# falcon-computing/falcon-genome

Hardware: AMD Instinct MI355X
Metric: PairHMM GCUPS + banded-SW GCUPS per GPU; end-to-end htc regions/sec at 8 GPUs (higher is better)
Workload: dtype fp32 (fp64 rescue)

## Files before the change

### falcon-genome_amd/csrc/phmm_cols.h

```cpp
#pragma once

namespace fcs {

constexpr int kColsClasses = 8;
constexpr int kColsMinR = 33;
__host__ __device__ constexpr int cols_C(int c) { return c == 0 ? 19 : 18 - c; }
__host__ __device__ constexpr int cols_hmax(int c) { return 16 * cols_C(c) - 1; }
__host__ __device__ inline int cols_class(int H) {
  for (int c = kColsClasses - 1; c >= 0; --c)
    if (H <= cols_hmax(c)) return c;
  return -1;
}
constexpr int kColsRing = 32;
constexpr int kColsChunks = 6;
constexpr int kColsChunkBytes = kColsRing * 4 * 16;
constexpr int kColsCapOff = kColsChunks * kColsChunkBytes;
constexpr int kColsTabOff = kColsCapOff + 4 * 8 * 8;
constexpr int kColsLds = kColsTabOff + 3 * 128 * 4;

__device__ __forceinline__ uint32_t vconst(uint32_t k) {
  uint32_t r;
  asm volatile("v_mov_b32 %0, %1" : "=v"(r) : "i"(k));
  return r;
}

struct ColsItem {
  float e1, e3, my, yy, mm, gm, mx, xx;
  uint32_t tlo, thi;
  float z;
};

__device__ __forceinline__ ColsItem cols_item(const PhmmTables<float>& tab, const RawRow& raw, int role, bool first,
                                              float ih) {
  ColsItem c;
  if (role == 2 || role == 3) {
    const RowP<float> q = row_params<float, false>(tab, raw);
    const float x0 = first ? ih * tab.dmatch[raw.gq & 127] : 1.f;
    const bool last = role == 3;
    c.e1 = q.e1 * x0;
    c.e3 = q.e3 * x0;
    c.my = last ? 0.f : q.my;
    c.yy = q.yy;
    c.mm = last ? 1.f : q.mm;
    c.gm = last ? 1.f : q.gm;
    c.mx = last ? 0.f : q.mx;
    c.xx = last ? 0.f : q.xx;
    const int bc = base_code((unsigned char)raw.rb);
    c.tlo = bc < 4 ? 1u << (8 * bc) : bc == 4 ? vconst(0x01010101u) : 0u;
    c.thi = 0x00000001u;
    c.z = 0.f;
  } else if (role == 4) {
    c.e1 = 1.f;
    c.e3 = 0.f;
    c.my = c.yy = c.mm = c.gm = 1.f;
    c.mx = c.xx = 0.f;
    c.tlo = vconst(0x01010101u);
    c.thi = vconst(0x00000101u);
    c.z = 0.f;
  } else {
    c.e1 = c.e3 = c.my = c.mm = c.gm = c.mx = c.xx = 0.f;
    c.yy = 1.f;
    c.tlo = c.thi = 0u;
    c.z = 1.f;
  }
  return c;
}

__device__ __forceinline__ void cols_put(unsigned char* smem, int slot, int seg, int h, const ColsItem& c) {
  float* const p = reinterpret_cast<float*>(smem + (seg * kColsRing + slot) * 16) + h;
  constexpr int F = kColsChunkBytes / 4;
  p[0] = c.e1;
  p[2] = c.e3;
  p[F] = c.my;
  p[F + 2] = c.yy;
  p[2 * F] = c.mm;
  p[2 * F + 2] = c.gm;
  p[3 * F] = c.mx;
  p[3 * F + 2] = c.xx;
  uint32_t* const q = reinterpret_cast<uint32_t*>(p);
  q[4 * F] = c.tlo;
  q[4 * F + 2] = c.thi;
  q[5 * F] = __float_as_uint(c.z);
  q[5 * F + 2] = __float_as_uint(c.z);
}

template <int NW>
__device__ __forceinline__ void cols_convert(const uint32_t (&raw)[NW + 1], int al, int i0, int H, uint32_t (&code)[NW],
                                             bool& other) {
#pragma unroll
  for (int d = 0; d < NW; ++d) {
    const uint32_t x = __builtin_amdgcn_alignbyte(raw[d + 1], raw[d], (uint32_t)al);
    const int rel = H - (i0 + 4 * d);
    const int nv = min(max(rel, 0), 4);
    const uint32_t vmask = nv >= 4 ? 0xFFFFFFFFu : (1u << (8 * nv)) - 1u;
    const uint32_t sel = (x >> 1) & vconst(0x07070707u);
    uint32_t c = __builtin_amdgcn_perm(vconst(0x04050505u), vconst(0x02030100u), sel);
    const uint32_t back = __builtin_amdgcn_perm(vconst(0x0000004Eu), vconst(0x54474341u), c);
    other |= ((back ^ x) & vmask) != 0u;
    c = (c & vmask) | (vconst(0x06060606u) & ~vmask);
    if (rel >= 0 && rel < 4) c = (c & ~(0xFFu << (8 * rel))) | (0x05u << (8 * rel));
    code[d] = c;
  }
}

template <int NW>
__device__ __forceinline__ void cols_load(const uint8_t* __restrict__ hb, int64_t ho, int H, int i0, uint32_t (&raw)[NW + 1],
                                          int& al) {
  const int64_t s = ho + i0;
  al = (int)(s & 3);
  const int64_t base = s - al;
  const uint32_t* const src = reinterpret_cast<const uint32_t*>(hb + base);
#pragma unroll
  for (int d = 0; d <= NW; ++d) raw[d] = (base + 4 * d < ho + H && H > 0) ? src[d] : 0u;
}

template <int C>
__global__ __launch_bounds__(64, 2) void phmm4_kernel(
    const PhmmDevBatch b, const int32_t* __restrict__ order, const int64_t* __restrict__ bounds, const int cls,
    const int K, const int tail_pairs, const PhmmTables<float> gtab, double* __restrict__ out,
    int32_t* __restrict__ rescue_list, unsigned long long* __restrict__ rescue_count, const float thr,
    const int use_rescue, int32_t* __restrict__ fb_list, unsigned long long* __restrict__ fb_count) {
  constexpr int NW = (C + 3) / 4;
  extern __shared__ __align__(16) unsigned char smem_raw[];
  const int lane = threadIdx.x;
  const int seg = lane >> 4;
  const int sl = lane & 15;
  const int sbase = lane & 48;
  const int th = sl >> 3, tk = sl & 7;
  const int i0 = sl * C;
  const int64_t cbeg = bounds[cls];
  const long long count = bounds[cls + 1] - cbeg;
  order += cbeg;
  PhmmTables<float> tab = gtab;
  {
    float* const t = reinterpret_cast<float*>(smem_raw + kColsTabOff);
    for (int i = lane; i < 128; i += 64) {
      t[i] = gtab.ph2pr[i];
      t[128 + i] = gtab.dmatch[i];
      t[256 + i] = gtab.dmis[i];
    }
    tab.ph2pr = t;
    tab.dmatch = t + 128;
    tab.dmis = t + 256;
  }
  const long long tailn = count < (long long)tail_pairs ? count : (long long)tail_pairs;
  const long long headn = count - tailn;
  const long long per = 8LL * K;
  const long long nb_head = (headn + per - 1) / per;
  const long long nbatch = nb_head + (tailn + 7) / 8;

  for (long long w = blockIdx.x; w < nbatch; w += gridDim.x) {
    const bool head = w < nb_head;
    const int Kb = head ? K : 1;
    const long long bstart = head ? w * per : headn + (w - nb_head) * 8;
    const long long bend = head ? min(headn, bstart + per) : min(count, bstart + 8);
    const long long idx = bstart + 2 * seg + th + 8LL * tk;
    const int pm = (tk < Kb && idx < bend) ? order[idx] : -1;
    int Rm = 0, Hm = 0;
    int64_t rom = 0, hom = 0;
    float Im = 0.f;
    if (pm >= 0) {
      const int ri = b.pair_read[pm], hi = b.pair_hap[pm];
      Rm = b.read_len[ri];
      Hm = b.hap_len[hi];
      rom = b.read_off[ri];
      hom = b.hap_off[hi];
      Im = tab.init_const / (float)Hm;
    }
    const int len = pm >= 0 ? Rm + 2 : 0;
    int incl = len;
#pragma unroll
    for (int d = 1; d < 8; d <<= 1) {
      const int v = __shfl_up(incl, d, 8);
      if (tk >= d) incl += v;
    }
    const int Gm = incl - len;
    const int totA = __builtin_amdgcn_ds_bpermute(4 * (sbase + 7), incl);
    const int totB = __builtin_amdgcn_ds_bpermute(4 * (sbase + 15), incl);
    const int nsteps = ((wave_max(max(totA, totB)) + 15) + 7) & ~7;
    int sb = sbase * 4;
    auto bp = [&](int v, int h, int k) {
      return __builtin_amdgcn_ds_bpermute(sb + 4 * (8 * h + min(k, 7)), v);
    };
    auto tG = [&](int h, int k) { return bp(Gm, h, k); };
    auto tR = [&](int h, int k) { return bp(Rm, h, k); };
    auto tH = [&](int h, int k) { return bp(Hm, h, k); };
    auto tP = [&](int h, int k) { return bp(pm, h, k); };
    auto tI = [&](int h, int k) { return __int_as_float(bp(__float_as_int(Im), h, k)); };
    auto t64 = [&](int64_t v, int h, int k) {
      const int lo = bp((int)v, h, k), hi = bp((int)(v >> 32), h, k);
      return (int64_t)(((uint64_t)(uint32_t)hi << 32) | (uint32_t)lo);
    };
    auto valid = [&](int h, int k) {
      const int pv = tP(h, k);
      return k < Kb && pv >= 0;
    };

    uint32_t cur[2][NW], nxt[2][NW];
    int nk[2], swr[2];
    unsigned other[2] = {0u, 0u};
    auto fetch_codes = [&](int h, int k, uint32_t (&dst)[NW]) {
      const bool ok = valid(h, k);
      const int Hk = tH(h, k);
      const int H = ok ? Hk : 0;
      const int64_t ho = t64(hom, h, k);
      uint32_t raw[NW + 1];
      int al;
      cols_load<NW>(b.hb, ok ? ho : 0, H, i0, raw, al);
      bool oth = false;
      cols_convert<NW>(raw, al, i0, H, dst, oth);
      const unsigned long long bal = __ballot(oth && ok);
      if (((bal >> sbase) & 0xFFFFull) != 0ull) other[h] |= 1u << k;
    };
#pragma unroll
    for (int h = 0; h < 2; ++h) {
#pragma unroll
      for (int d = 0; d < NW; ++d) cur[h][d] = 0x06060606u;
      fetch_codes(h, 0, nxt[h]);
      nk[h] = 0;
      swr[h] = valid(h, 0) ? tG(h, 0) : 0x3FFFFFFF;
    }
    int kc[2] = {0, 0};
    int cap[2], capp[2];
    auto load_cap = [&](int h) {
      const bool ok = valid(h, kc[h]);
      const int v = tG(h, kc[h]) + tR(h, kc[h]);
      cap[h] = ok ? v : -0x3FFFFFFF;
      capp[h] = tP(h, kc[h]);
    };
    load_cap(0);
    load_cap(1);

    int kp = 0;
    RawRow praw{-1, 0, 0, 0, 0, 0, 0};
    int prole = 0;
    float pih = 0.f;
    bool kok = false, nok = false;
    int kG = 0, kR = 0, nG = 0;
    float kI = 0.f;
    int64_t kro = 0;
    auto load_cursor = [&] {
      kok = valid(th, kp);
      kG = tG(th, kp);
      kR = tR(th, kp);
      kI = tI(th, kp);
      kro = t64(rom, th, kp);
      nok = valid(th, kp + 1);
      nG = tG(th, kp + 1);
    };
    load_cursor();
    auto stage_a = [&](int base) {
      const int g = base + tk;
      const bool adv = nok && g >= nG;
      if (__ballot(adv) != 0ull) {
        if (adv) ++kp;
        load_cursor();
      }
      const bool ok = kok;
      const int G = kG, R = kR;
      pih = kI;
      const int64_t ro = kro;
      const int r = g - G;
      int role = 0;
      if (ok && r >= 0 && r < R) role = r == R - 1 ? 3 : 2;
      else if (ok && r == R) role = 4;
      prole = role | (r == 0 ? 16 : 0);
      praw = (role == 2 || role == 3) ? load_raw(b, R, ro, r) : RawRow{-1, 0, 0, 0, 0, 0, 0};
    };
    auto stage_b = [&](int base) {
      cols_put(smem_raw, (base + tk) & (kColsRing - 1), seg, th,
               cols_item(tab, praw, prole & 15, (prole & 16) != 0, pih));
    };
    {
      ColsItem z = cols_item(tab, RawRow{-1, 0, 0, 0, 0, 0, 0}, 0, false, 0.f);
      cols_put(smem_raw, 16 + tk, seg, th, z);
      cols_put(smem_raw, 24 + tk, seg, th, z);
      stage_a(0);
      stage_b(0);
      stage_a(8);
    }

    pf2 Xn[C], In[C];
#pragma unroll
    for (int j = 0; j < C; ++j) {
      Xn[j] = pf2{1.f, 1.f};
      In[j] = pf2{0.f, 0.f};
    }
    pf2 dn = pf2{1.f, 1.f}, xo = pf2{1.f, 1.f}, xin = pf2{1.f, 1.f};
    const uint32_t segoff = (uint32_t)seg * (kColsRing * 16u) + lds_addr(smem_raw);

    for (int t0 = 0; t0 < nsteps; t0 += 8) {
      asm volatile("" : "+v"(sb));
#pragma unroll
      for (int h = 0; h < 2; ++h) {
        const bool ev = swr[h] + 16 <= t0 && nk[h] + 1 < Kb;
        if (__ballot(ev) != 0ull) {
          uint32_t tmp[NW];
          fetch_codes(h, nk[h] + 1, tmp);
          const bool vn = valid(h, nk[h] + 1);
          const int gn = tG(h, nk[h] + 1);
          if (ev) {
#pragma unroll
            for (int d = 0; d < NW; ++d) nxt[h][d] = tmp[d];
            ++nk[h];
            swr[h] = vn ? gn : 0x3FFFFFFF;
          }
        }
        if (swr[h] + 16 <= t0 && nk[h] + 1 >= Kb) swr[h] = 0x3FFFFFFF;
      }
      stage_b(t0 + 8);
      stage_a(t0 + 16);
#pragma unroll
      for (int h = 0; h < 2; ++h) {
        const bool adv = cap[h] >= 0 && cap[h] + 15 < t0;
        if (__ballot(adv) != 0ull) {
          if (adv) ++kc[h];
          load_cap(h);
        }
      }
      bool capo[2];
#pragma unroll
      for (int h = 0; h < 2; ++h) capo[h] = (other[h] >> kc[h]) & 1u;
      const int g0 = t0 - sl;
      const bool any_cap = __ballot(sl == 15 && ((unsigned)(cap[0] - g0) < 8u || (unsigned)(cap[1] - g0) < 8u)) != 0ull;
      unsigned swmask = 0u;
#pragma unroll
      for (int q = 0; q < 4; ++q)
#pragma unroll
        for (int h = 0; h < 2; ++h) {
          const int lo = __builtin_amdgcn_readlane(swr[h], 16 * q) - t0;
          if (lo < 8 && lo + 15 >= 0) {
            const int a = max(lo, 0), bnd = min(lo + 15, 7);
            swmask |= ((2u << bnd) - 1u) & ~((1u << a) - 1u);
          }
        }
      const uint32_t xs = (uint32_t)(g0 & (kColsRing - 1)) * 16u;
      const uint32_t capa = lds_addr(smem_raw) + kColsCapOff + seg * 64;

      auto step = [&](auto S_) {
        constexpr int S = decltype(S_)::value;
        const int g = g0 + S;
        if (swmask & (1u << S)) {
#pragma unroll
          for (int h = 0; h < 2; ++h) {
            const bool take = g == swr[h];
#pragma unroll
            for (int d = 0; d < NW; ++d) {
              uint32_t r;
              asm("v_cndmask_b32_e64 %0, %1, %2, %3" : "=v"(r) : "v"(cur[h][d]), "v"(nxt[h][d]), "s"(__ballot(take)));
              cur[h][d] = r;
            }
          }
        }
        asm volatile("" ::: "memory");
        const uint32_t pa = ((xs + (uint32_t)(S * 16)) & (uint32_t)((kColsRing - 1) * 16)) + segoff;
        typedef float f4 __attribute__((ext_vector_type(4)));
        typedef uint32_t u4 __attribute__((ext_vector_type(4)));
        auto ld4 = [&](int chunk) {
          return *reinterpret_cast<const __attribute__((address_space(3))) f4*>((uintptr_t)(pa + chunk * kColsChunkBytes));
        };
        const f4 r0 = ld4(0), r1 = ld4(1), r2 = ld4(2), r3 = ld4(3);
        const u4 cr = *reinterpret_cast<const __attribute__((address_space(3))) u4*>((uintptr_t)(pa + 4 * kColsChunkBytes));
        const pf2 z1 = *reinterpret_cast<const __attribute__((address_space(3))) pf2*>((uintptr_t)(pa + 5 * kColsChunkBytes));
        const pf2 z2 = *reinterpret_cast<const __attribute__((address_space(3))) pf2*>((uintptr_t)(pa + 5 * kColsChunkBytes + 8));
        const pf2 e1 = pf2{r0.x, r0.y}, e3 = pf2{r0.z, r0.w}, my = pf2{r1.x, r1.y}, yy = pf2{r1.z, r1.w};
        const pf2 mm = pf2{r2.x, r2.y}, gm = pf2{r2.z, r2.w}, mx = pf2{r3.x, r3.y}, xx = pf2{r3.z, r3.w};
        pf2 din, xnx;
        din.x = __int_as_float(__builtin_amdgcn_update_dpp(__float_as_int(z1.x), __float_as_int(dn.x), kDppRowShr1, 0xF, 0xF, false));
        din.y = __int_as_float(__builtin_amdgcn_update_dpp(__float_as_int(z1.y), __float_as_int(dn.y), kDppRowShr1, 0xF, 0xF, false));
        xnx.x = __int_as_float(__builtin_amdgcn_update_dpp(__float_as_int(z2.x), __float_as_int(xo.x), kDppRowShr1, 0xF, 0xF, false));
        xnx.y = __int_as_float(__builtin_amdgcn_update_dpp(__float_as_int(z2.y), __float_as_int(xo.y), kDppRowShr1, 0xF, 0xF, false));
        const pf2 xcur = xin;
        xin = xnx;
        uint32_t mA = 0, mB = 0;
        auto prior = [&](int j, const pf2 dep) {
          if ((j & 3) == 0) {
            mA = __builtin_amdgcn_perm(cr.z, cr.x, cur[0][j >> 2]);
            mB = __builtin_amdgcn_perm(cr.w, cr.y, cur[1][j >> 2]);
          }
          int a, c;
          asm volatile("v_bfe_i32 %0, %2, %3, 1\n\tv_bfe_i32 %1, %4, %3, 1"
                       : "=&v"(a), "=&v"(c)
                       : "v"(mA), "i"(8 * (j & 3)), "v"(mB), "v"(dep));
          return pf2{sel_v((uint32_t)a, e1.x, e3.x), sel_v((uint32_t)c, e1.y, e3.y)};
        };
        pf2 Mn = xcur * prior(0, xcur);
        pf2 D = din, Mp = pf2{0.f, 0.f}, Dp = pf2{0.f, 0.f};
#pragma unroll
        for (int j = 0; j < C; ++j) {
          const pf2 M = Mn;
          if (j > 0) D = __builtin_elementwise_fma(Mp, my, Dp * yy);
          pf2 I = In[j], Xo = Xn[j];
          asm volatile("" : "+v"(I), "+v"(Xo) : "v"(D));
          if (j + 1 < C) Mn = Xo * prior(j + 1, D);
          pf2 xn = __builtin_elementwise_fma(M, mm, __builtin_elementwise_fma(I, gm, D));
          pf2 in = __builtin_elementwise_fma(M, mx, I * xx);
          asm volatile("" : "+v"(xn), "+v"(in));
          Xn[j] = xn;
          In[j] = in;
          Mp = M;
          Dp = D;
        }
        dn = __builtin_elementwise_fma(Mp, my, Dp * yy);
        xo = Xn[C - 1];
        uint64_t keep;
        const uint32_t cpa = capa + 0u;
        const pf2 dnv = dn;
        asm volatile(
            "s_mov_b64 %0, exec\n\t"
            "s_mov_b64 exec, %3\n\t"
            "ds_write_b64 %1, %2 offset:%4\n\t"
            "s_mov_b64 exec, %0"
            : "=&s"(keep)
            : "v"(cpa), "v"(dnv), "s"(kTopLanes), "i"(8 * S)
            : "memory");
      };
      [&]<int... S>(std::integer_sequence<int, S...>) {
        (step(std::integral_constant<int, S>{}), ...);
      }(std::make_integer_sequence<int, 8>{});
      if (any_cap) {
#pragma unroll
        for (int h = 0; h < 2; ++h)
          if (sl == 15 && (unsigned)(cap[h] - g0) < 8u) {
            const pf2 v = *reinterpret_cast<const pf2*>(smem_raw + kColsCapOff + seg * 64 + 8 * (cap[h] - g0));
            const float acc = h ? v.y : v.x;
            const int p = capp[h];
            if (capo[h]) {
              const unsigned long long k = atomicAdd(fb_count, 1ull);
              fb_list[k] = p;
              out[p] = __builtin_nan("");
            } else if (use_rescue && acc < thr) {
              const unsigned long long k = atomicAdd(rescue_count, 1ull);
              rescue_list[k] = p;
              out[p] = __builtin_nan("");
            } else {
              out[p] = (double)(log10f(acc) - tab.log10_init);
            }
          }
      }
    }
  }
}

constexpr int kCols1Ring = 48;
constexpr int kCols1Chunks = 5;
constexpr int kCols1ChunkBytes = kCols1Ring * 4 * 8;
constexpr int kCols1CapOff = kCols1Chunks * kCols1ChunkBytes;
constexpr int kCols1TabOff = kCols1CapOff + 4 * 16 * 4;
constexpr int kCols1Lds = kCols1TabOff + 3 * 128 * 4;
constexpr int kCols1MaxK = 16;
__host__ __device__ constexpr int cols1_waves(int C) { return 3; }
static_assert(kCols1Lds <= 10240, "16 waves per CU");

typedef uint32_t pu2 __attribute__((ext_vector_type(2)));

__device__ __forceinline__ void cols1_put(unsigned char* smem, int slot, int seg, const ColsItem& c) {
  unsigned char* const p = smem + (seg * kCols1Ring + slot) * 8;
  *reinterpret_cast<pf2*>(p) = pf2{c.e1, c.e3};
  *reinterpret_cast<pf2*>(p + kCols1ChunkBytes) = pf2{c.my, c.yy};
  *reinterpret_cast<pf2*>(p + 2 * kCols1ChunkBytes) = pf2{c.mm, c.gm};
  *reinterpret_cast<pf2*>(p + 3 * kCols1ChunkBytes) = pf2{c.mx, c.xx};
  *reinterpret_cast<pu2*>(p + 4 * kCols1ChunkBytes) = pu2{c.tlo, c.thi | (c.z != 0.f ? 0x01000000u : 0u)};
}

constexpr int kNever = 0x3FFFFFFF;

struct Cols1Seg {
  int pm, Rm, Hm, Gm;
  int64_t rom, hom;
  float Im;
};

__device__ __forceinline__ PhmmTables<float> cols1_tables(const PhmmTables<float>& gtab) {
  extern __shared__ __align__(16) unsigned char smem_raw[];
  PhmmTables<float> tab = gtab;
  float* const t = reinterpret_cast<float*>(smem_raw + kCols1TabOff);
  for (int i = threadIdx.x; i < 128; i += 64) {
    t[i] = gtab.ph2pr[i];
    t[128 + i] = gtab.dmatch[i];
    t[256 + i] = gtab.dmis[i];
  }
  tab.ph2pr = t;
  tab.dmatch = t + 128;
  tab.dmis = t + 256;
  return tab;
}

struct Cols1Batch {
  static constexpr bool kQueue = false;
  int Kb, nsteps;
  static __device__ __forceinline__ int slot(int k) { return min(k, 15); }
  static __device__ __forceinline__ int bit(int k) { return k; }
  __device__ __forceinline__ bool more(int t0) const { return t0 < nsteps; }
  __device__ __forceinline__ bool done(int) const { return false; }
};

constexpr int kCols6Lds = kCols1Lds;
constexpr int kCols6Waves = 3;
constexpr int kCols6Ahead = 48;
static_assert(kCols6Lds <= 13653, "12 waves per CU");

struct Cols1Queue {
  static constexpr bool kQueue = true;
  const int32_t* order;
  long long count;
  unsigned long long* qhead;
  unsigned pend;
  uint32_t qv;
  int nq = 0, gend = 0;
  bool closed = false;
  static __device__ __forceinline__ int slot(int k) { return k & 15; }
  static __device__ __forceinline__ int bit(int k) { return k & 15; }
  __device__ __forceinline__ bool more(int) const { return true; }
  __device__ __forceinline__ bool done(int kc) const { return __ballot(!closed || kc < nq) == 0ull; }
  __device__ __forceinline__ void complete(int gmin, const PhmmDevBatch& b, const PhmmTables<float>& tab, Cols1Seg& tb,
                                           unsigned& other) {
    const int seg = threadIdx.x >> 4, sl = threadIdx.x & 15;
    const long long base = (long long)(uint32_t)__builtin_amdgcn_readfirstlane((int)qv);
    const bool mine = (pend >> seg) & 1u;
    const long long idx = base + __popc(pend & ((1u << seg) - 1u));
    const bool got = mine && idx < count;
    if (mine && !got) closed = true;
    if (got) {
      const int p = order[idx];
      const int ri = b.pair_read[p], hi = b.pair_hap[p];
      const int R = b.read_len[ri], H = b.hap_len[hi];
      const int G = max(gend, gmin);
      if (sl == (nq & 15)) {
        tb.pm = p;
        tb.Rm = R;
        tb.Hm = H;
        tb.rom = b.read_off[ri];
        tb.hom = b.hap_off[hi];
        tb.Im = tab.init_const / (float)H;
        tb.Gm = G;
      }
      other &= ~(1u << (nq & 15));
      gend = G + R + 2;
      ++nq;
    }
    pend = 0u;
  }
  __device__ __forceinline__ void request(int t0, int kc) {
    const bool need = !closed && gend < t0 + 32 + kCols6Ahead && nq - kc < 8;
    const unsigned long long bal = __ballot(need && (threadIdx.x & 15) == 0);
    if (bal != 0ull) {
      pend = (unsigned)((bal & 1ull) | ((bal >> 15) & 2ull) | ((bal >> 30) & 4ull) | ((bal >> 45) & 8ull));
      qv = 0u;
      if (threadIdx.x == 0) qv = (uint32_t)atomicAdd(qhead, (unsigned long long)__popc(pend));
    }
  }
};

template <int C, class Feed>
__device__ __forceinline__ void cols1_stream(const PhmmDevBatch& b, const PhmmTables<float>& tab, Cols1Seg tb,
                                             Feed feed, double* __restrict__ out,
                                             int32_t* __restrict__ rescue_list,
                                             unsigned long long* __restrict__ rescue_count, const float thr,
                                             const int use_rescue, int32_t* __restrict__ fb_list,
                                             unsigned long long* __restrict__ fb_count) {
  constexpr int NW = (C + 3) / 4;
  extern __shared__ __align__(16) unsigned char smem_raw[];
  const int lane = threadIdx.x;
  const int seg = lane >> 4;
  const int sl = lane & 15;
  const int sbase = lane & 48;
  const int i0 = sl * C;
  int sb = sbase * 4;
  auto bp = [&](int v, int k) { return __builtin_amdgcn_ds_bpermute(sb + 4 * Feed::slot(k), v); };
  auto tG = [&](int k) { return bp(tb.Gm, k); };
  auto tR = [&](int k) { return bp(tb.Rm, k); };
  auto tH = [&](int k) { return bp(tb.Hm, k); };
  auto tP = [&](int k) { return bp(tb.pm, k); };
  auto tI = [&](int k) { return __int_as_float(bp(__float_as_int(tb.Im), k)); };
  auto t64 = [&](int64_t v, int k) {
    const int lo = bp((int)v, k), hi = bp((int)(v >> 32), k);
    return (int64_t)(((uint64_t)(uint32_t)hi << 32) | (uint32_t)lo);
  };
  auto valid = [&](int k) {
    if constexpr (Feed::kQueue) {
      return k >= 0 && k < feed.nq;
    } else {
      const int pv = tP(k);
      return k < feed.Kb && pv >= 0;
    }
  };

  uint32_t cur[NW], nxt[NW];
  int nk = -1, swr = kNever;
  unsigned other = 0u;
  auto fetch_codes = [&](int k, uint32_t (&dst)[NW]) {
    const bool ok = valid(k);
    const int Hk = tH(k);
    const int H = ok ? Hk : 0;
    const int64_t ho = t64(tb.hom, k);
    uint32_t raw[NW + 1];
    int al;
    cols_load<NW>(b.hb, ok ? ho : 0, H, i0, raw, al);
    bool oth = false;
    cols_convert<NW>(raw, al, i0, H, dst, oth);
    const unsigned long long bal = __ballot(oth && ok);
    if (((bal >> sbase) & 0xFFFFull) != 0ull) other |= 1u << Feed::bit(k);
  };
#pragma unroll
  for (int d = 0; d < NW; ++d) cur[d] = nxt[d] = 0x06060606u;
  int kc = 0, cap, capp;
  auto load_cap = [&] {
    const bool ok = valid(kc);
    const int v = tG(kc) + tR(kc);
    cap = ok ? v : -kNever;
    capp = tP(kc);
  };

  int kp = 0;
  RawRow praw{-1, 0, 0, 0, 0, 0, 0};
  int prole = 0;
  float pih = 0.f;
  bool kok = false, nok = false;
  int kG = 0, kR = 0, nG = 0;
  float kI = 0.f;
  int64_t kro = 0;
  auto load_cursor = [&] {
    kok = valid(kp);
    kG = tG(kp);
    kR = tR(kp);
    kI = tI(kp);
    kro = t64(tb.rom, kp);
    nok = valid(kp + 1);
    nG = tG(kp + 1);
  };
  auto stage_a = [&](int base) {
    const int g = base + sl;
    const bool adv = nok && g >= nG;
    if (__ballot(adv) != 0ull) {
      if (adv) ++kp;
      load_cursor();
    }
    const int r = g - kG;
    int role = 0;
    if (kok && r >= 0 && r < kR) role = r == kR - 1 ? 3 : 2;
    else if (kok && r == kR) role = 4;
    pih = kI;
    prole = role | (r == 0 ? 16 : 0);
    praw = (role == 2 || role == 3) ? load_raw(b, kR, kro, r) : RawRow{-1, 0, 0, 0, 0, 0, 0};
  };
  auto stage_b = [&](int base) {
    cols1_put(smem_raw, (int)((unsigned)(base + sl) % (unsigned)kCols1Ring), seg,
              cols_item(tab, praw, prole & 15, (prole & 16) != 0, pih));
  };
  if constexpr (Feed::kQueue) {
    feed.complete(0, b, tab, tb, other);
  } else {
    fetch_codes(0, nxt);
    nk = 0;
    swr = valid(0) ? tG(0) : kNever;
  }
  load_cursor();
  load_cap();
  {
    cols1_put(smem_raw, 32 + sl, seg, cols_item(tab, RawRow{-1, 0, 0, 0, 0, 0, 0}, 0, false, 0.f));
    stage_a(0);
    stage_b(0);
    stage_a(16);
  }

  float Xn[C], In[C];
#pragma unroll
  for (int j = 0; j < C; ++j) {
    Xn[j] = 1.f;
    In[j] = 0.f;
  }
  float dn = 1.f, xo = 1.f, xin = 1.f;
  const uint32_t segoff = (uint32_t)seg * (kCols1Ring * 8u) + lds_addr(smem_raw);

  for (int t0 = 0; feed.more(t0); t0 += 16) {
    asm volatile("" : "+v"(sb));
    if constexpr (Feed::kQueue) {
      if (feed.pend != 0u) {
        feed.complete(t0 + 32, b, tab, tb, other);
        load_cursor();
        load_cap();
      }
      feed.request(t0, kc);
    }
    {
      bool ev;
      if constexpr (Feed::kQueue) {
        if (swr != kNever && swr + 16 <= t0) swr = kNever;
        ev = swr == kNever && nk + 1 < feed.nq;
      } else {
        ev = swr + 16 <= t0 && nk + 1 < feed.Kb;
      }
      if (__ballot(ev) != 0ull) {
        uint32_t tmp[NW];
        fetch_codes(nk + 1, tmp);
        const bool vn = valid(nk + 1);
        const int gn = tG(nk + 1);
        if (ev) {
#pragma unroll
          for (int d = 0; d < NW; ++d) nxt[d] = tmp[d];
          ++nk;
          swr = vn ? gn : kNever;
        }
      }
      if constexpr (!Feed::kQueue)
        if (swr + 16 <= t0 && nk + 1 >= feed.Kb) swr = kNever;
    }
    stage_b(t0 + 16);
    stage_a(t0 + 32);
    {
      const bool adv = cap >= 0 && cap + 15 < t0;
      if (__ballot(adv) != 0ull) {
        if (adv) ++kc;
        load_cap();
      }
    }
    if (feed.done(kc)) break;
    const bool capo = (other >> Feed::bit(kc)) & 1u;
    const int gb = t0 - sl;
    const bool any_cap = __ballot(sl == 15 && (unsigned)(cap - gb) < 16u) != 0ull;
    unsigned swmask = 0u;
#pragma unroll
    for (int q = 0; q < 4; ++q) {
      const int lo = __builtin_amdgcn_readlane(swr, 16 * q) - t0;
      if (lo < 16 && lo + 15 >= 0) {
        const int a = max(lo, 0), bnd = min(lo + 15, 15);
        swmask |= ((2u << bnd) - 1u) & ~((1u << a) - 1u);
      }
    }
    uint32_t xs = ((uint32_t)(gb + kCols1Ring) % (uint32_t)kCols1Ring) * 8u;
    uint32_t capa = lds_addr(smem_raw) + kCols1CapOff + seg * 64;
    int g0 = gb;

#pragma nounroll
    for (int pass = 0; pass < 2; ++pass) {
      auto step = [&](auto S_) {
        constexpr int S = decltype(S_)::value;
        const int g = g0 + S;
        if (swmask & (1u << S)) {
          const bool take = g == swr;
#pragma unroll
          for (int d = 0; d < NW; ++d) {
            uint32_t r;
            asm("v_cndmask_b32_e64 %0, %1, %2, %3" : "=v"(r) : "v"(cur[d]), "v"(nxt[d]), "s"(__ballot(take)));
            cur[d] = r;
          }
        }
        asm volatile("" ::: "memory");
        const uint32_t a0 = xs + (uint32_t)(S * 8);
        const uint32_t pa = min(a0, a0 - (uint32_t)(kCols1Ring * 8)) + segoff;
        auto ld2 = [&](int chunk) {
          return *reinterpret_cast<const __attribute__((address_space(3))) pf2*>((uintptr_t)(pa + chunk * kCols1ChunkBytes));
        };
        const pf2 r0 = ld2(0), r1 = ld2(1), r2 = ld2(2), r3 = ld2(3);
        const pu2 cr = *reinterpret_cast<const __attribute__((address_space(3))) pu2*>((uintptr_t)(pa + 4 * kCols1ChunkBytes));
        const float e1 = r0.x, e3 = r0.y, my = r1.x, yy = r1.y, mm = r2.x, gm = r2.y, mx = r3.x, xx = r3.y;
        const float z = (float)(cr.y >> 24);
        const float din = __int_as_float(__builtin_amdgcn_update_dpp(__float_as_int(z), __float_as_int(dn), kDppRowShr1, 0xF, 0xF, false));
        const float xnx = __int_as_float(__builtin_amdgcn_update_dpp(__float_as_int(z), __float_as_int(xo), kDppRowShr1, 0xF, 0xF, false));
        const float xcur = xin;
        xin = xnx;
        uint32_t mA = 0;
        auto prior = [&](int j, const float dep) {
          if ((j & 3) == 0) mA = __builtin_amdgcn_perm(cr.y, cr.x, cur[j >> 2]);
          int a;
          asm volatile("v_bfe_i32 %0, %1, %2, 1" : "=v"(a) : "v"(mA), "i"(8 * (j & 3)), "v"(dep));
          return sel_v((uint32_t)a, e1, e3);
        };
        float Mn = xcur * prior(0, xcur);
        float D = din, Mp = 0.f, Dp = 0.f;
#pragma unroll
        for (int j = 0; j < C; ++j) {
          const float M = Mn;
          if (j > 0) D = __builtin_fmaf(Mp, my, Dp * yy);
          float I = In[j], Xo = Xn[j];
          asm volatile("" : "+v"(I), "+v"(Xo) : "v"(D));
          if (j + 1 < C) Mn = Xo * prior(j + 1, D);
          float xn = __builtin_fmaf(M, mm, __builtin_fmaf(I, gm, D));
          float in = __builtin_fmaf(M, mx, I * xx);
          asm volatile("" : "+v"(xn), "+v"(in));
          Xn[j] = xn;
          In[j] = in;
          Mp = M;
          Dp = D;
        }
        dn = __builtin_fmaf(Mp, my, Dp * yy);
        xo = Xn[C - 1];
        uint64_t keep;
        const uint32_t cpa = capa + 0u;
        const float dnv = dn;
        asm volatile(
            "s_mov_b64 %0, exec\n\t"
            "s_mov_b64 exec, %3\n\t"
            "ds_write_b32 %1, %2 offset:%4\n\t"
            "s_mov_b64 exec, %0"
            : "=&s"(keep)
            : "v"(cpa), "v"(dnv), "s"(kTopLanes), "i"(4 * S)
            : "memory");
      };
      [&]<int... S>(std::integer_sequence<int, S...>) {
        (step(std::integral_constant<int, S>{}), ...);
      }(std::make_integer_sequence<int, 8>{});
      g0 += 8;
      swmask >>= 8;
      capa += 32;
      xs += 64;
      xs = min(xs, xs - (uint32_t)(kCols1Ring * 8));
    }
    if (any_cap) {
      if (sl == 15 && (unsigned)(cap - gb) < 16u) {
        const float acc = *reinterpret_cast<const float*>(smem_raw + kCols1CapOff + seg * 64 + 4 * (cap - gb));
        const int p = capp;
        if (capo) {
          const unsigned long long k = atomicAdd(fb_count, 1ull);
          fb_list[k] = p;
          out[p] = __builtin_nan("");
        } else if (use_rescue && acc < thr) {
          const unsigned long long k = atomicAdd(rescue_count, 1ull);
          rescue_list[k] = p;
          out[p] = __builtin_nan("");
        } else {
          out[p] = (double)(log10f(acc) - tab.log10_init);
        }
      }
    }
  }
}

template <int C>
__global__ __launch_bounds__(64, cols1_waves(C)) void phmm5_kernel(
    const PhmmDevBatch b, const int32_t* __restrict__ order, const int64_t* __restrict__ bounds, const int cls,
    const int K, const int tail_pairs, const PhmmTables<float> gtab, double* __restrict__ out,
    int32_t* __restrict__ rescue_list, unsigned long long* __restrict__ rescue_count, const float thr,
    const int use_rescue, int32_t* __restrict__ fb_list, unsigned long long* __restrict__ fb_count) {
  const int lane = threadIdx.x;
  const int seg = lane >> 4;
  const int sl = lane & 15;
  const int sbase = lane & 48;
  const int64_t cbeg = bounds[cls];
  const long long count = bounds[cls + 1] - cbeg;
  order += cbeg;
  const PhmmTables<float> tab = cols1_tables(gtab);
  const long long tailn = count < (long long)tail_pairs ? count : (long long)tail_pairs;
  const long long headn = count - tailn;
  const long long per = 4LL * K;
  const long long nb_head = (headn + per - 1) / per;
  const long long nbatch = nb_head + (tailn + 3) / 4;

  for (long long w = blockIdx.x; w < nbatch; w += gridDim.x) {
    const bool head = w < nb_head;
    const int Kb = head ? K : 1;
    const long long bstart = head ? w * per : headn + (w - nb_head) * 4;
    const long long bend = head ? min(headn, bstart + per) : min(count, bstart + 4);
    const long long idx = bstart + seg + 4LL * sl;
    Cols1Seg tb{(sl < Kb && idx < bend) ? order[idx] : -1, 0, 0, 0, 0, 0, 0.f};
    if (tb.pm >= 0) {
      const int ri = b.pair_read[tb.pm], hi = b.pair_hap[tb.pm];
      tb.Rm = b.read_len[ri];
      tb.Hm = b.hap_len[hi];
      tb.rom = b.read_off[ri];
      tb.hom = b.hap_off[hi];
      tb.Im = tab.init_const / (float)tb.Hm;
    }
    const int len = tb.pm >= 0 ? tb.Rm + 2 : 0;
    int incl = len;
#pragma unroll
    for (int d = 1; d < 16; d <<= 1) {
      const int v = __shfl_up(incl, d, 16);
      if (sl >= d) incl += v;
    }
    tb.Gm = incl - len;
    const int tot = __builtin_amdgcn_ds_bpermute(4 * (sbase + 15), incl);
    const int nsteps = ((wave_max(tot) + 15) + 15) & ~15;
    cols1_stream<C>(b, tab, tb, Cols1Batch{Kb, nsteps}, out, rescue_list, rescue_count, thr, use_rescue, fb_list,
                    fb_count);
  }
}

template <int C>
__global__ __launch_bounds__(64, kCols6Waves) void phmm6_kernel(
    const PhmmDevBatch b, const int32_t* __restrict__ order, const int64_t* __restrict__ bounds, const int cls,
    const PhmmTables<float> gtab, double* __restrict__ out, int32_t* __restrict__ rescue_list,
    unsigned long long* __restrict__ rescue_count, const float thr, const int use_rescue,
    int32_t* __restrict__ fb_list, unsigned long long* __restrict__ fb_count,
    unsigned long long* __restrict__ qhead) {
  const int64_t cbeg = bounds[cls];
  const long long count = bounds[cls + 1] - cbeg;
  uint32_t qv = 0u;
  if (threadIdx.x == 0) qv = (uint32_t)atomicAdd(qhead, 4ull);
  if ((long long)(uint32_t)__builtin_amdgcn_readfirstlane((int)qv) >= count) return;
  const PhmmTables<float> tab = cols1_tables(gtab);
  cols1_stream<C>(b, tab, Cols1Seg{-1, 0, 0, 0, 0, 0, 0.f}, Cols1Queue{order + cbeg, count, qhead, 0xFu, qv}, out,
                  rescue_list, rescue_count, thr, use_rescue, fb_list, fb_count);
}

}
```

Measured before the change: 4584.

## Rescale PairHMM column recurrence by mm to drop one multiply per cell

```diff
diff --git a/falcon-genome_amd/csrc/phmm_cols.h b/falcon-genome_amd/csrc/phmm_cols.h
--- a/falcon-genome_amd/csrc/phmm_cols.h
+++ b/falcon-genome_amd/csrc/phmm_cols.h
@@ -25,24 +25,30 @@
 }
 
 struct ColsItem {
-  float e1, e3, my, yy, mm, gm, mx, xx;
+  float e1, e3, b, yy, a, mx, xx;
   uint32_t tlo, thi;
   float z;
 };
 
-__device__ __forceinline__ ColsItem cols_item(const PhmmTables<float>& tab, const RawRow& raw, int role, bool first,
-                                              float ih) {
+constexpr float kColsMinMm = 0.0625f;
+
+__device__ __forceinline__ ColsItem cols_item(const PhmmTables<float>& tab, const RawRow& raw, int oiq, int role,
+                                              bool first, float ih, bool& hazard) {
   ColsItem c;
+  hazard = false;
   if (role == 2 || role == 3) {
     const RowP<float> q = row_params<float, false>(tab, raw);
-    const float x0 = first ? ih * tab.dmatch[raw.gq & 127] : 1.f;
+    const int oi = oiq & 127, od = raw.dq & 127;
+    const int hi = oi > od ? oi : od, lo = oi > od ? od : oi;
+    const float x0 = first ? ih * tab.dmatch[raw.gq & 127] : tab.mm[((hi * (hi + 1)) >> 1) + lo];
     const bool last = role == 3;
+    hazard = !last && !(q.mm >= kColsMinMm);
+    const float inv = (last || hazard) ? 0.f : 1.f / q.mm;
     c.e1 = q.e1 * x0;
     c.e3 = q.e3 * x0;
-    c.my = last ? 0.f : q.my;
+    c.b = q.my * inv;
     c.yy = q.yy;
-    c.mm = last ? 1.f : q.mm;
-    c.gm = last ? 1.f : q.gm;
+    c.a = last ? 1.f : q.gm * inv;
     c.mx = last ? 0.f : q.mx;
     c.xx = last ? 0.f : q.xx;
     const int bc = base_code((unsigned char)raw.rb);
@@ -52,14 +58,14 @@
   } else if (role == 4) {
     c.e1 = 1.f;
     c.e3 = 0.f;
-    c.my = c.yy = c.mm = c.gm = 1.f;
-    c.mx = c.xx = 0.f;
+    c.yy = 1.f;
+    c.a = c.b = c.mx = c.xx = 0.f;
     c.tlo = vconst(0x01010101u);
     c.thi = vconst(0x00000101u);
     c.z = 0.f;
   } else {
-    c.e1 = c.e3 = c.my = c.mm = c.gm = c.mx = c.xx = 0.f;
-    c.yy = 1.f;
+    c.e1 = c.e3 = c.a = c.mx = c.xx = 0.f;
+    c.b = c.yy = 1.f;
     c.tlo = c.thi = 0u;
     c.z = 1.f;
   }
@@ -71,10 +77,10 @@
   constexpr int F = kColsChunkBytes / 4;
   p[0] = c.e1;
   p[2] = c.e3;
-  p[F] = c.my;
+  p[F] = c.b;
   p[F + 2] = c.yy;
-  p[2 * F] = c.mm;
-  p[2 * F + 2] = c.gm;
+  p[2 * F] = c.a;
+  p[2 * F + 2] = 0.f;
   p[3 * F] = c.mx;
   p[3 * F + 2] = c.xx;
   uint32_t* const q = reinterpret_cast<uint32_t*>(p);
@@ -266,13 +272,23 @@
       else if (ok && r == R) role = 4;
       prole = role | (r == 0 ? 16 : 0);
       praw = (role == 2 || role == 3) ? load_raw(b, R, ro, r) : RawRow{-1, 0, 0, 0, 0, 0, 0};
+      if (role == 2 || role == 3) prole |= (int)b.iq[ro + r] << 8;
     };
     auto stage_b = [&](int base) {
+      bool hz;
       cols_put(smem_raw, (base + tk) & (kColsRing - 1), seg, th,
-               cols_item(tab, praw, prole & 15, (prole & 16) != 0, pih));
+               cols_item(tab, praw, prole >> 8, prole & 15, (prole & 16) != 0, pih, hz));
+      if (__ballot(hz) != 0ull) {
+        unsigned m = hz ? 1u << (kp + 8 * th) : 0u;
+#pragma unroll
+        for (int d = 1; d < 16; d <<= 1) m |= (unsigned)__shfl_xor((int)m, d, 16);
+        other[0] |= m & 0xFFu;
+        other[1] |= m >> 8;
+      }
     };
     {
-      ColsItem z = cols_item(tab, RawRow{-1, 0, 0, 0, 0, 0, 0}, 0, false, 0.f);
+      bool hz;
+      ColsItem z = cols_item(tab, RawRow{-1, 0, 0, 0, 0, 0, 0}, 0, 0, false, 0.f, hz);
       cols_put(smem_raw, 16 + tk, seg, th, z);
       cols_put(smem_raw, 24 + tk, seg, th, z);
       stage_a(0);
@@ -363,8 +379,8 @@
         const u4 cr = *reinterpret_cast<const __attribute__((address_space(3))) u4*>((uintptr_t)(pa + 4 * kColsChunkBytes));
         const pf2 z1 = *reinterpret_cast<const __attribute__((address_space(3))) pf2*>((uintptr_t)(pa + 5 * kColsChunkBytes));
         const pf2 z2 = *reinterpret_cast<const __attribute__((address_space(3))) pf2*>((uintptr_t)(pa + 5 * kColsChunkBytes + 8));
-        const pf2 e1 = pf2{r0.x, r0.y}, e3 = pf2{r0.z, r0.w}, my = pf2{r1.x, r1.y}, yy = pf2{r1.z, r1.w};
-        const pf2 mm = pf2{r2.x, r2.y}, gm = pf2{r2.z, r2.w}, mx = pf2{r3.x, r3.y}, xx = pf2{r3.z, r3.w};
+        const pf2 e1 = pf2{r0.x, r0.y}, e3 = pf2{r0.z, r0.w}, cb = pf2{r1.x, r1.y}, yy = pf2{r1.z, r1.w};
+        const pf2 ca = pf2{r2.x, r2.y}, mx = pf2{r3.x, r3.y}, xx = pf2{r3.z, r3.w};
         pf2 din, xnx;
         din.x = __int_as_float(__builtin_amdgcn_update_dpp(__float_as_int(z1.x), __float_as_int(dn.x), kDppRowShr1, 0xF, 0xF, false));
         din.y = __int_as_float(__builtin_amdgcn_update_dpp(__float_as_int(z1.y), __float_as_int(dn.y), kDppRowShr1, 0xF, 0xF, false));
@@ -385,23 +401,23 @@
           return pf2{sel_v((uint32_t)a, e1.x, e3.x), sel_v((uint32_t)c, e1.y, e3.y)};
         };
         pf2 Mn = xcur * prior(0, xcur);
-        pf2 D = din, Mp = pf2{0.f, 0.f}, Dp = pf2{0.f, 0.f};
+        pf2 E = din, Mp = pf2{0.f, 0.f}, Ep = pf2{0.f, 0.f};
 #pragma unroll
         for (int j = 0; j < C; ++j) {
           const pf2 M = Mn;
-          if (j > 0) D = __builtin_elementwise_fma(Mp, my, Dp * yy);
+          if (j > 0) E = __builtin_elementwise_fma(Ep, yy, Mp);
           pf2 I = In[j], Xo = Xn[j];
-          asm volatile("" : "+v"(I), "+v"(Xo) : "v"(D));
-          if (j + 1 < C) Mn = Xo * prior(j + 1, D);
-          pf2 xn = __builtin_elementwise_fma(M, mm, __builtin_elementwise_fma(I, gm, D));
+          asm volatile("" : "+v"(I), "+v"(Xo) : "v"(E));
+          if (j + 1 < C) Mn = Xo * prior(j + 1, E);
+          pf2 xn = __builtin_elementwise_fma(E, cb, __builtin_elementwise_fma(I, ca, M));
           pf2 in = __builtin_elementwise_fma(M, mx, I * xx);
           asm volatile("" : "+v"(xn), "+v"(in));
           Xn[j] = xn;
           In[j] = in;
           Mp = M;
-          Dp = D;
+          Ep = E;
         }
-        dn = __builtin_elementwise_fma(Mp, my, Dp * yy);
+        dn = __builtin_elementwise_fma(Ep, yy, Mp);
         xo = Xn[C - 1];
         uint64_t keep;
         const uint32_t cpa = capa + 0u;
@@ -457,8 +473,8 @@
 __device__ __forceinline__ void cols1_put(unsigned char* smem, int slot, int seg, const ColsItem& c) {
   unsigned char* const p = smem + (seg * kCols1Ring + slot) * 8;
   *reinterpret_cast<pf2*>(p) = pf2{c.e1, c.e3};
-  *reinterpret_cast<pf2*>(p + kCols1ChunkBytes) = pf2{c.my, c.yy};
-  *reinterpret_cast<pf2*>(p + 2 * kCols1ChunkBytes) = pf2{c.mm, c.gm};
+  *reinterpret_cast<pf2*>(p + kCols1ChunkBytes) = pf2{c.b, c.yy};
+  *reinterpret_cast<pf2*>(p + 2 * kCols1ChunkBytes) = pf2{c.a, 0.f};
   *reinterpret_cast<pf2*>(p + 3 * kCols1ChunkBytes) = pf2{c.mx, c.xx};
   *reinterpret_cast<pu2*>(p + 4 * kCols1ChunkBytes) = pu2{c.tlo, c.thi | (c.z != 0.f ? 0x01000000u : 0u)};
 }
@@ -643,10 +659,18 @@
     pih = kI;
     prole = role | (r == 0 ? 16 : 0);
     praw = (role == 2 || role == 3) ? load_raw(b, kR, kro, r) : RawRow{-1, 0, 0, 0, 0, 0, 0};
+    if (role == 2 || role == 3) prole |= (int)b.iq[kro + r] << 8;
   };
   auto stage_b = [&](int base) {
+    bool hz;
     cols1_put(smem_raw, (int)((unsigned)(base + sl) % (unsigned)kCols1Ring), seg,
-              cols_item(tab, praw, prole & 15, (prole & 16) != 0, pih));
+              cols_item(tab, praw, prole >> 8, prole & 15, (prole & 16) != 0, pih, hz));
+    if (__ballot(hz) != 0ull) {
+      unsigned m = hz ? 1u << Feed::bit(kp) : 0u;
+#pragma unroll
+      for (int d = 1; d < 16; d <<= 1) m |= (unsigned)__shfl_xor((int)m, d, 16);
+      other |= m;
+    }
   };
   if constexpr (Feed::kQueue) {
     feed.complete(0, b, tab, tb, other);
@@ -658,7 +682,8 @@
   load_cursor();
   load_cap();
   {
-    cols1_put(smem_raw, 32 + sl, seg, cols_item(tab, RawRow{-1, 0, 0, 0, 0, 0, 0}, 0, false, 0.f));
+    bool hz;
+    cols1_put(smem_raw, 32 + sl, seg, cols_item(tab, RawRow{-1, 0, 0, 0, 0, 0, 0}, 0, 0, false, 0.f, hz));
     stage_a(0);
     stage_b(0);
     stage_a(16);
@@ -752,9 +777,10 @@
         auto ld2 = [&](int chunk) {
           return *reinterpret_cast<const __attribute__((address_space(3))) pf2*>((uintptr_t)(pa + chunk * kCols1ChunkBytes));
         };
-        const pf2 r0 = ld2(0), r1 = ld2(1), r2 = ld2(2), r3 = ld2(3);
+        const pf2 r0 = ld2(0), r1 = ld2(1), r3 = ld2(3);
+        const float ca = *reinterpret_cast<const __attribute__((address_space(3))) float*>((uintptr_t)(pa + 2 * kCols1ChunkBytes));
         const pu2 cr = *reinterpret_cast<const __attribute__((address_space(3))) pu2*>((uintptr_t)(pa + 4 * kCols1ChunkBytes));
-        const float e1 = r0.x, e3 = r0.y, my = r1.x, yy = r1.y, mm = r2.x, gm = r2.y, mx = r3.x, xx = r3.y;
+        const float e1 = r0.x, e3 = r0.y, cb = r1.x, yy = r1.y, mx = r3.x, xx = r3.y;
         const float z = (float)(cr.y >> 24);
         const float din = __int_as_float(__builtin_amdgcn_update_dpp(__float_as_int(z), __float_as_int(dn), kDppRowShr1, 0xF, 0xF, false));
         const float xnx = __int_as_float(__builtin_amdgcn_update_dpp(__float_as_int(z), __float_as_int(xo), kDppRowShr1, 0xF, 0xF, false));
@@ -768,23 +794,23 @@
           return sel_v((uint32_t)a, e1, e3);
         };
         float Mn = xcur * prior(0, xcur);
-        float D = din, Mp = 0.f, Dp = 0.f;
+        float E = din, Mp = 0.f, Ep = 0.f;
 #pragma unroll
         for (int j = 0; j < C; ++j) {
           const float M = Mn;
-          if (j > 0) D = __builtin_fmaf(Mp, my, Dp * yy);
+          if (j > 0) E = __builtin_fmaf(Ep, yy, Mp);
           float I = In[j], Xo = Xn[j];
-          asm volatile("" : "+v"(I), "+v"(Xo) : "v"(D));
-          if (j + 1 < C) Mn = Xo * prior(j + 1, D);
-          float xn = __builtin_fmaf(M, mm, __builtin_fmaf(I, gm, D));
+          asm volatile("" : "+v"(I), "+v"(Xo) : "v"(E));
+          if (j + 1 < C) Mn = Xo * prior(j + 1, E);
+          float xn = __builtin_fmaf(E, cb, __builtin_fmaf(I, ca, M));
           float in = __builtin_fmaf(M, mx, I * xx);
           asm volatile("" : "+v"(xn), "+v"(in));
           Xn[j] = xn;
           In[j] = in;
           Mp = M;
-          Dp = D;
+          Ep = E;
         }
-        dn = __builtin_fmaf(Mp, my, Dp * yy);
+        dn = __builtin_fmaf(Ep, yy, Mp);
         xo = Xn[C - 1];
         uint64_t keep;
         const uint32_t cpa = capa + 0u;
```

Result: faster. 4765 (median of 6 runs) (+3.9%).
